# flysoaryun/LF-VIO

Measured on AMD Instinct MI355X. Metric: sliding-window solves/sec (10 KF x N landmarks), higher is better.
Workload: dtype f64; 1 GPU; window300; landmarks=300, observations=1419, windows_per_gpu=1, marginalization=MARGIN_OLD, parallelism=1 independent window stream(s), one per GPU, no data-path collective

## Files before the change

### lf-vio_amd/csrc/kernels_marg.h

```cpp
#pragma once
#include "kernels_solve.h"

constexpr int MARG_THREADS = 768;
constexpr int MARG_MAXD = 96;
constexpr int LDN = 80;
constexpr double JACOBI_TOL = 1e-19;
constexpr size_t MARG_LDS = (size_t)19072 * sizeof(double);
constexpr int BT_GROUP = 4;

DEV void gauge_landmarks(Slot *S, int l0) {
  const int l = l0 + (int)threadIdx.x;
  double *lam = S->lam[S->tr.cur];
  if (l < S->N) lam[l] = 1.0 / (1.0 / lam[l]);
}
template <class T>
DEV void copy_rounds(T *dst, const T *src, int n, int tid, int nthr) {
  for (int k0 = tid; k0 < n; k0 += 8 * nthr) {
    T v[8];
#pragma unroll
    for (int q = 0; q < 8; q++) v[q] = src[k0 + q * nthr < n ? k0 + q * nthr : 0];
#pragma unroll
    for (int q = 0; q < 8; q++)
      if (k0 + q * nthr < n) dst[k0 + q * nthr] = v[q];
  }
}
DEV void gauge_poses(Slot *S, int gated, bool publish);
DEV void publish_solution(Slot *S) {
  char *m = (char *)S->mail;
  if (!m) return;
  const int tid = threadIdx.x, nthr = blockDim.x;
  const TRState *ts = &S->tr;
  const int cur = ts->cur, N = S->N;
  {
    constexpr int XW = (int)(sizeof(FrameState) / 8), XT = (XW + 63) / 64, LT = (SPEC_MAX_LM + 63) / 64, TT = 8;
    const double *xs = (const double *)&S->x[cur];
    double *xd = (double *)(m + MAIL_X + (size_t)cur * sizeof(FrameState));
    const long long *tsrc = (const long long *)ts;
    long long *tdst = (long long *)(m + MAIL_TR);
    const int tl = ts->trace_len < LFVIO_MAX_TRACE ? ts->trace_len : LFVIO_MAX_TRACE;
    const int words = (int)((offsetof(TRState, trace) + (size_t)(tl > 0 ? tl : 0) * sizeof(LfvioIterationSummary)) / 8);
    const double *ls = S->lam[cur];
// ... 426 lines not shown
  unsigned cnt = (unsigned)__double2hiint(p) >> 31;
  unsigned bits = (unsigned)__double2hiint(p) >> 31;
  double d0[8], e0[8], d1[8], e1[8];
#pragma unroll
  for (int u = 0; u < 8; u++) d0[u] = Tg[1 + u], e0[u] = Tg[96 + u];
  for (int i0 = 1; i0 < n; i0 += 16) {
    STURM_TOUCH8(d0);
    STURM_TOUCH8(e0);
#pragma unroll
    for (int u = 0; u < 8; u++) d1[u] = Tg[i0 + 8 + u], e1[u] = Tg[96 + i0 + 8 + u - 1];
#pragma unroll
    for (int u = 0; u < 8; u++) {
      const double pn = fma(d0[u] - sigma, p, -e0[u] * pm);
      bits = __builtin_amdgcn_alignbit(bits, (unsigned)__double2hiint(pn), 31);
      pm = p, p = pn;
    }
    STURM_TOUCH8(d1);
    STURM_TOUCH8(e1);
#pragma unroll
    for (int u = 0; u < 8; u++) d0[u] = Tg[i0 + 16 + u], e0[u] = Tg[96 + i0 + 16 + u - 1];
#pragma unroll
    for (int u = 0; u < 8; u++) {
      const double pn = fma(d1[u] - sigma, p, -e1[u] * pm);
      bits = __builtin_amdgcn_alignbit(bits, (unsigned)__double2hiint(pn), 31);
      pm = p, p = pn;
    }
    cnt += __builtin_popcount((bits ^ (bits >> 1)) & 0xffffu);
    const int ex = ilogb(fmax(fmax(fabs(p), fabs(pm)), 1e-300));
    p = ldexp(p, -ex), pm = ldexp(pm, -ex);
  }
  return (int)cnt;
}
struct TriCtx {
  double *dd, *ee, *tau, *vb0, *vb1, *pp, *RV;
  int n, r0, c0;
};
template <int P>
DEV void tri_finish_row(const TriCtx &tc, int kk, const double (&row)[5], bool own) {
  const int n = tc.n, c0 = tc.c0;
  double *vb = (kk & 1) ? tc.vb1 : tc.vb0;
  double a_part = 0.0, ss_part = 0.0, dk = 0.0;
  bool has_d = false;
#pragma unroll
  for (int q = P; q < 5; q++) {
    const int C = c0 + 16 * q;
    if (C == kk) dk = row[q], has_d = true;
    if (C == kk + 1) a_part = row[q];
    if (C > kk + 1 && C < n) ss_part = fma(row[q], row[q], ss_part);
  }
  if (own && has_d) tc.dd[kk] = dk;
  if (kk + 2 >= n) {
    if (own && kk == n - 2 && c0 == ((n - 1) & 15)) tc.ee[kk] = a_part;
    return;
  }
  a_part = sum8(a_part), ss_part = sum8(ss_part);
  const double alpha = a_part + dpp_f64<0x140>(a_part), ss = ss_part + dpp_f64<0x140>(ss_part);
  const double nn = fma(alpha, alpha, ss);
  const bool live = ss > 0.0;
  const double rs = fast_rsqrt(live ? nn : 1.0);
  const double beta = live ? -copysign(nn * rs, alpha) : alpha;
  const double t = live ? (beta - alpha) * -copysign(rs, alpha) : 0.0;
  const double scal = live ? fast_rcp(alpha - beta) : 0.0;
  if (own) {
#pragma unroll
    for (int q = P; q < 5; q++) {
      const int C = c0 + 16 * q;
      const double v = C == kk + 1 ? 1.0 : ((C > kk + 1 && C < n) ? row[q] * scal : 0.0);
      vb[C] = v;
      if (C > kk && C < n) tc.RV[kk * 76 + C - kk - 1] = v;
    }
    if (c0 == 0) tc.tau[kk] = t, tc.ee[kk] = beta;
  }
}
template <int P>
DEV void tri_matvec(const TriCtx &tc, int k, const double (&ar)[5][5], double (&vj)[5]) {
  const double *vb = (k & 1) ? tc.vb1 : tc.vb0;
  const double t = tc.tau[k];
#pragma unroll
  for (int q = P; q < 5; q++) vj[q] = vb[tc.c0 + 16 * q];
  double sacc[5];
#pragma unroll
  for (int i = P; i < 5; i++) {
    sacc[i] = 0.0;
#pragma unroll
    for (int q = P; q < 5; q++) sacc[i] = fma(ar[i][q], vj[q], sacc[i]);
  }
#pragma unroll
  for (int i = P; i < 5; i++) sacc[i] += dpp_f64<0xB1>(sacc[i]);
#pragma unroll
  for (int i = P; i < 5; i++) sacc[i] += dpp_f64<0x4E>(sacc[i]);
#pragma unroll
  for (int i = P; i < 5; i++) sacc[i] += dpp_f64<0x141>(sacc[i]);
#pragma unroll
  for (int i = P; i < 5; i++) sacc[i] += dpp_f64<0x140>(sacc[i]);
  if (tc.c0 == 0) {
#pragma unroll
    for (int i = P; i < 5; i++) tc.pp[tc.r0 + 16 * i] = tc.r0 + 16 * i > k ? t * sacc[i] : 0.0;
  }
}
template <int P>
DEV void tri_update(const TriCtx &tc, int k, double (&ar)[5][5], const double (&vj)[5]) {
  const double *vb = (k & 1) ? tc.vb1 : tc.vb0;
  const double t = tc.tau[k];
  double pj[5], vi[5], pi[5], pvs = 0.0;
#pragma unroll
  for (int q = P; q < 5; q++) pj[q] = tc.pp[tc.c0 + 16 * q];
#pragma unroll
  for (int i = P; i < 5; i++) vi[i] = vb[tc.r0 + 16 * i], pi[i] = tc.pp[tc.r0 + 16 * i];
#pragma unroll
  for (int q = P; q < 5; q++) pvs = fma(pj[q], vj[q], pvs);
  pvs = sum8(pvs);
  pvs += dpp_f64<0x140>(pvs);
  const double K2 = t * pvs;
#pragma unroll
  for (int i = P; i < 5; i++) {
#pragma unroll
    for (int q = P; q < 5; q++) ar[i][q] = fma(-pi[i], vj[q], fma(-vi[i], pj[q], ar[i][q]));
  }
#pragma unroll
  for (int i = P; i < 5; i++) {
    const double kv = K2 * vi[i];
#pragma unroll
    for (int q = P; q < 5; q++) ar[i][q] = fma(kv, vj[q], ar[i][q]);
    if (i == P) tri_finish_row<P>(tc, k + 1, ar[P], tc.r0 == ((k + 1) & 15));
  }
}
template <int QM, int NR>
DEV void bt_apply(const double *RV, const double *tau, int k, int n, int l8, double (&zz)[10]) {
  double vq[NR][10], tk[NR];
#pragma unroll
  for (int r = 0; r < NR; r++) {
    const int kr = k - r;
    const double *v = RV + kr * 76 - (kr + 1);
    tk[r] = tau[kr];
#pragma unroll
    for (int q = QM; q < 10; q++) {
      const int i = l8 + 8 * q;
      if (QM == 0) vq[r][q] = (i > kr && i < n) ? v[i] : 0.0;
      else vq[r][q] = (q > QM || i > kr) ? v[i] : 0.0;
    }
  }
#pragma unroll
  for (int r = 0; r < NR; r++) {
    double s0 = 0.0, s1 = 0.0;
#pragma unroll
    for (int q = QM; q < 10; q++) {
      if ((q - QM) & 1) s1 = fma(vq[r][q], zz[q], s1);
      else s0 = fma(vq[r][q], zz[q], s0);
    }
    const double s = sum8(s0 + s1) * tk[r];
#pragma unroll
    for (int q = QM; q < 10; q++) zz[q] = fma(-s, vq[r][q], zz[q]);
  }
}
template <int NR>
DEV void bt_dispatch(const double *RV, const double *tau, int k, int n, int l8, double (&zz)[10]) {
  switch (k >> 3) {
    case 0: bt_apply<0, NR>(RV, tau, k, n, l8, zz); break;
    case 1: bt_apply<1, NR>(RV, tau, k, n, l8, zz); break;
    case 2: bt_apply<2, NR>(RV, tau, k, n, l8, zz); break;
    case 3: bt_apply<3, NR>(RV, tau, k, n, l8, zz); break;
    case 4: bt_apply<4, NR>(RV, tau, k, n, l8, zz); break;
    case 5: bt_apply<5, NR>(RV, tau, k, n, l8, zz); break;
    case 6: bt_apply<6, NR>(RV, tau, k, n, l8, zz); break;
    case 7: bt_apply<7, NR>(RV, tau, k, n, l8, zz); break;
    case 8: bt_apply<8, NR>(RV, tau, k, n, l8, zz); break;
    default: bt_apply<9, NR>(RV, tau, k, n, l8, zz); break;
  }
}
DEV double guard_pivot(double q, double pivmin) { return copysign(fmax(fabs(q), pivmin), q); }
template <bool SPEC>
DEV bool eig_tridiag(double *A, const double *b, int n, int tid, double *RV, double *DM, double *vec, double *scr, double *nn2, double *Tglob, LfvioPrior *out, double eps, long long *dbg,
                     SpecPoll *sp_) {
  SpecPoll *const sp = SPEC ? sp_ : nullptr;
  const bool poller = SPEC && tid == MARG_THREADS - 1;
#define ESTAMP(k) do { if (tid == 0) dbg[k] = (long long)__builtin_readcyclecounter(); } while (0)
  ESTAMP(26);
  const int wave = tid >> 6, lane = tid & 63;
  double *dd = vec, *ee = vec + 96, *ee2 = vec + 192, *tau = vec + 288, *lam = vec + 384, *pp = vec + 480, *nrm = vec + 576;
  const bool tri = tid < 256;
  const int r0 = (tid >> 4) & 15, c0 = tid & 15;
  double ar[5][5];
#pragma unroll
  for (int i = 0; i < 5; i++)
#pragma unroll
    for (int q = 0; q < 5; q++) {
      const int R = r0 + 16 * i, C = c0 + 16 * q;
      ar[i][q] = (tri && R < n && C < n) ? A[max(R, C) * LDN + min(R, C)] : 0.0;
    }
  double *vb0 = lam, *vb1 = nrm;
  if (tid < 96) dd[tid] = 0.0, ee[tid] = 0.0, ee2[tid] = 0.0, tau[tid] = 0.0, vb0[tid] = 0.0, vb1[tid] = 0.0;
  for (int e = tid; e < 76 * 76; e += MARG_THREADS) RV[e] = 0.0;
  __syncthreads();
  TriCtx tc = {dd, ee, tau, vb0, vb1, pp, RV, n, r0, c0};
  if (tri) tri_finish_row<0>(tc, 0, ar[0], r0 == 0);
  __syncthreads();
  for (int k = 0; k + 2 < n; k++) {
    const int P = (k + 1) >> 4;
    double vj[5];
    if (poller) {
      if ((k & 7) == 0) spec_poll_issue(*sp);
      else if ((k & 7) == 6) spec_poll_take(*sp);
    }
#ifdef LFVIO_TRI_PROFILE
#define TSTAMP(j) do { if (tid == 0 && k == LFVIO_TRI_PROFILE) dbg[3 + j] = (long long)__builtin_readcyclecounter(); } while (0)
#else
#define TSTAMP(j) do { } while (0)
#endif
    TSTAMP(0);
    if (tri) {
      switch (P) {
        case 0: tri_matvec<0>(tc, k, ar, vj); break;
        case 1: tri_matvec<1>(tc, k, ar, vj); break;
        case 2: tri_matvec<2>(tc, k, ar, vj); break;
        case 3: tri_matvec<3>(tc, k, ar, vj); break;
        default: tri_matvec<4>(tc, k, ar, vj); break;
      }
    }
    TSTAMP(1);
    __syncthreads();
    TSTAMP(2);
    if (tri) {
      switch (P) {
        case 0: tri_update<0>(tc, k, ar, vj); break;
        case 1: tri_update<1>(tc, k, ar, vj); break;
        case 2: tri_update<2>(tc, k, ar, vj); break;
        case 3: tri_update<3>(tc, k, ar, vj); break;
        default: tri_update<4>(tc, k, ar, vj); break;
      }
    }
    TSTAMP(3);
    __syncthreads();
    TSTAMP(4);
    if (sp && (k & 7) == 6 && *sp->flag) return true;
  }
  if (tri) {
#pragma unroll
    for (int i = 0; i < 5; i++)
#pragma unroll
      for (int q = 0; q < 5; q++)
        if (r0 + 16 * i == n - 1 && c0 + 16 * q == n - 1) dd[n - 1] = ar[i][q];
  }
  if (poller) spec_poll_issue(*sp);
  __syncthreads();
  ESTAMP(27);
  if (tid < n) ee2[tid] = ee[tid] * ee[tid];
  {
    double lo = 1e300, hi = -1e300;
    if (tid < n) {
      const double r = (tid > 0 ? fabs(ee[tid - 1]) : 0.0) + (tid + 1 < n ? fabs(ee[tid]) : 0.0);
      lo = dd[tid] - r, hi = dd[tid] + r;
    }
    lo = -wave_max(-lo), hi = wave_max(hi);
    if (lane == 0) scr[wave] = lo, scr[16 + wave] = hi;
  }
  __syncthreads();
  double gl = fmin(scr[0], scr[1]), gu = fmax(scr[16], scr[17]);
  {
    const double tn = fmax(fabs(gl), fabs(gu));
    gl -= 2.2e-16 * tn * n + 1e-300, gu += 2.2e-16 * tn * n + 1e-300;
  }
  if (tid < 96) Tglob[tid] = tid < n ? dd[tid] : gu + 1.0, Tglob[96 + tid] = tid + 1 < n ? ee[tid] * ee[tid] : 0.0;
  __threadfence();
  __syncthreads();
  __builtin_amdgcn_s_dcache_inv();
  const unsigned long long ta = (unsigned long long)Tglob;
  unsigned tlo = __builtin_amdgcn_readfirstlane((unsigned)ta), thi = __builtin_amdgcn_readfirstlane((unsigned)(ta >> 32));
  asm volatile("" : "+s"(tlo), "+s"(thi));
  sdouble *Tg = (sdouble *)(((unsigned long long)thi << 32) | tlo);
  {
    const double pivmin = 1e-290;
    const int g3 = lane == 63 ? 20 : lane / 3, l8 = lane == 63 ? 3 : lane - 3 * g3;
    const int m = wave * 21 + g3;
    const int mm = m < n ? m : n - 1;
    {
      int *cntg = (int *)pp;
      double *blo = nn2, *bhi = nn2 + 96;
      const double step = (gu - gl) * (1.0 / 257.0);
      if (tid < 96) blo[tid] = gl, bhi[tid] = gu;
      if (tid < 256) cntg[tid] = sturm_count(Tg, n, gl + step * (double)(tid + 1));
      __syncthreads();
      if (tid <= 256) {
        const int c0 = tid > 0 ? cntg[tid - 1] : 0, c1 = tid < 256 ? cntg[tid] : n;
        const double a = tid > 0 ? gl + step * (double)tid : gl, b = tid < 256 ? gl + step * (double)(tid + 1) : gu;
        for (int e = max(c0, 0); e < min(c1, n); e++) blo[e] = a, bhi[e] = b;
      }
      __syncthreads();
    }
    double lo = nn2[mm], hi = nn2[96 + mm];
    if (tid < 256)
      for (int round = 0; round < 23; round++) {
        const double w = hi - lo;
        const double sigma = lo + w * (double)(l8 < 3 ? l8 + 1 : 1) * 0.25;
        const int cnt = sturm_count(Tg, n, sigma);
        const int f1 = cnt <= mm ? 1 : 0;
        const unsigned long long bal = __ballot(f1);
        const int f = __builtin_popcount((unsigned)(bal >> (3 * g3)) & 7u);
        const double nlo = f == 0 ? lo : lo + w * (double)f * 0.25, nhi = f == 3 ? hi : lo + w * (double)(f + 1) * 0.25;
        lo = nlo, hi = nhi;
      }
    if (tid < 256 && m < n && l8 == 0) lam[m] = 0.5 * (lo + hi);
    if (poller) spec_poll_take(*sp), spec_poll_issue(*sp);
    __syncthreads();
    ESTAMP(28);
    if (sp && *sp->flag) return true;
    const int set = tid >> 7, me = tid & 127;
    const bool work = set < 2 && me < n;
    const int mec = work ? me : 0;
    const double l = lam[mec];
    if (work && set == 0) {
      double q = dd[0] - l;
      A[mec] = q;
      for (int i0 = 1; i0 < n; i0 += 8) {
        double dv[8], ev[8], qs[8];
#pragma unroll
        for (int u = 0; u < 8; u++) dv[u] = dd[i0 + u], ev[u] = ee2[i0 + u - 1];
#pragma unroll
        for (int u = 0; u < 8; u++) {
          q = fma(-ev[u], fast_rcp(guard_pivot(q, pivmin)), dv[u] - l);
          qs[u] = q;
        }
#pragma unroll
        for (int u = 0; u < 8; u++)
// ... 59 lines not shown
            zs[u] = z;
            nn = on ? fma(z, z, nn) : nn;
          }
#pragma unroll
          for (int u = 0; u < 8; u++)
            if (i0 - u < kt && i0 - u >= 0) A[(i0 - u) * LDN + mec] = zs[u];
        }
      } else {
        for (int i0 = 1; i0 < n; i0 += 8) {
          double c[8], zs[8];
#pragma unroll
          for (int u = 0; u < 8; u++) {
            const int i = min(i0 + u, n - 1);
            c[u] = -ee[i - 1] * fast_rcp(guard_pivot(DM[i * LDN + mec], pivmin));
          }
#pragma unroll
          for (int u = 0; u < 8; u++) {
            const bool on = i0 + u > kt && i0 + u < n;
            z = on ? c[u] * z : 1.0;
            zs[u] = z;
            nn = on ? fma(z, z, nn) : nn;
          }
#pragma unroll
          for (int u = 0; u < 8; u++)
            if (i0 + u > kt && i0 + u < n) A[(i0 + u) * LDN + mec] = zs[u];
        }
      }
      nn2[set * 96 + mec] = nn;
    }
  }
  __syncthreads();
  ESTAMP(29);
  {
    const int m = tid >> 3, l8 = tid & 7;
    const bool live = m < n;
    const int mm = live ? m : 0;
    double zz[10];
    const double sc = fast_rsqrt(1.0 + nn2[mm] + nn2[96 + mm]);
#pragma unroll
    for (int q = 0; q < 10; q++) {
      const int i = l8 + 8 * q;
      zz[q] = i < n ? A[i * LDN + mm] * sc : 0.0;
    }
    int k = n - 3;
    for (; k >= 0 && (k & (BT_GROUP - 1)) != BT_GROUP - 1; k--) bt_dispatch<1>(RV, tau, k, n, l8, zz);
    for (; k >= 0; k -= BT_GROUP) bt_dispatch<BT_GROUP>(RV, tau, k, n, l8, zz);
    const double l = lam[mm];
    double rb = 0.0;
#pragma unroll
    for (int q = 0; q < 10; q++) {
      const int i = l8 + 8 * q;
      if (i < n) rb = fma(zz[q], b[i], rb);
    }
    rb = sum8(rb);
    if (live) {
      const bool keep = l > eps;
      const double sq = keep ? sqrt(l) : 0.0;
#pragma unroll
      for (int q = 0; q < 10; q++) {
        const int i = l8 + 8 * q;
        if (i < n) out->linearized_jacobians[m * n + i] = sq * zz[q];
      }
      if (l8 == 0) out->linearized_residuals[m] = keep ? rb / sq : 0.0;
    }
  }
  return false;
}

DEV void spec_deliver(Slot *S, Slot *S0, int my_word, bool publish) {
  const int tid = threadIdx.x, nthr = blockDim.x;
  __shared__ int give;
  if (tid == 0) {
    const int ep = spec_ep(my_word), a = spec_acc(my_word);
    long long t0 = wall_clock64();
    int g = 0;
    for (;;) {
      const int f = spec_peek(&S0->spec.fin), w = spec_peek(&S0->spec.word);
      if (spec_ep(w) != ep) break;
      const int st = spec_ep(f) == ep ? spec_fin_state(f) : FIN_OPEN;
      if (st >= FIN_MAIN) {
        g = st == FIN_SIDE && spec_fin_acc(f) == a;
        break;
      }
      if (w != my_word) break;
      if (wall_clock64() - t0 > SPEC_WAIT_TICKS) {
        if (spec_cas(&S0->spec.own[a], SPEC_SIDE, SPEC_ABANDON) == SPEC_SIDE) break;
        t0 = wall_clock64();
      }
      __builtin_amdgcn_s_sleep(8);
    }
    give = g;
  }
  __syncthreads();
  if (!give) return;
  const LfvioPrior *src = &S->prior_out;
  LfvioPrior *dst = &S0->prior_out;
// ... 18 lines not shown
  const int publish = (flag_bits >> 10) & 1;
  constexpr bool worker = WORKER;
  Slot *S = worker ? (Slot *)base : SLOT(base, stride);
  Slot *S0 = worker ? (Slot *)(base - stride) : S;
  __shared__ int spec_flag;
  SpecPoll sp{S0, worker ? S->shadow.word : 0, &spec_flag, 0, 0};
  if (threadIdx.x == 0) spec_flag = 0;
  const bool poller = worker && threadIdx.x == MARG_THREADS - 1;
  TRState *tr = &S->tr;
  const MargPlan *mp = &S->marg[flag];
  const int tid = threadIdx.x;
  LfvioPrior *out = &S->prior_out;
  if (gated && !tail_gate(S, tr->done)) return;
  if (worker && sp.my_word == 0) return;
  if (!mp->valid) {
    if (tid == 0) out->valid = -1;
    if (worker) {
      __syncthreads();
      spec_deliver(S, S0, sp.my_word, publish != 0);
      return;
    }
    if (gated && tid == 0) S->iters_done = tr->iteration, S->tail_state = 2;
    if (gated && publish) {
      __syncthreads();
      publish_prior(S);
    }
    return;
  }
  if (poller) spec_poll_issue(sp);
  STAMP(S, 10);
  const double *Sc = S->schur_sum;
  const bool sub = mp->N0 > 0 || S->sharded;
  const int m15 = mp->m15, n = mp->n, D = m15 + n;
  double *Ag = S->mscr;
  double *A = smem;
  double *bv = A + 92 * 92;
  double *Am = bv + 96;
  double *Vm = Am + 256;
  double *Ainv = Vm + 256;
  double *Tm = Ainv + 256;
  double *Ar = smem + 12544;
  double *br = Ar + 76 * LDN;
  double2 *cs = (double2 *)(br + 80);
  int *perm = (int *)(cs + 96);
  double *scr = (double *)(perm + 96);
  double *RV = smem, *vec8 = smem + 5776, *DMs = smem + 5776 + 672;
  for (int c = tid; c < KP; c += MARG_THREADS) {
    const int a = mp->col[c];
    if (a >= 0) perm[a] = c;
  }
  __syncthreads();
  {
    constexpr int GR = (92 * 92 + MARG_THREADS - 1) / MARG_THREADS;
    const double *Hp = &S->Hpp[0];
    double hv[GR], sv[GR];
#pragma unroll
    for (int k = 0; k < GR; k++) {
      const int e = tid + MARG_THREADS * k, ec = e < D * D ? e : 0;
      const int r = D ? perm[ec / max(D, 1)] : 0, c = D ? perm[ec % max(D, 1)] : 0;
      const int hi = max(r, c), lo = min(r, c);
      hv[k] = Hp[hi * (hi + 1) / 2 + lo];
      sv[k] = (sub && hi < KC) ? Sc[schur_index(lo, hi)] : 0.0;
    }
#pragma unroll
    for (int k = 0; k < GR; k++) {
      const int e = tid + MARG_THREADS * k;
      if (e < D * D) A[e] = hv[k] - sv[k];
// ... 45 lines not shown
  }
  __syncthreads();
  {
    const int nb4 = (n + 3) >> 2;
    for (int blk = tid; blk < nb4 * nb4; blk += MARG_THREADS) {
      const int r0 = 4 * (blk / nb4), c0 = 4 * (blk % nb4);
      double acc[4][4];
#pragma unroll
      for (int i = 0; i < 4; i++)
#pragma unroll
        for (int j = 0; j < 4; j++) acc[i][j] = 0.0;
      for (int k = 0; k < m15; k++) {
        double tv[4], av[4];
#pragma unroll
        for (int i = 0; i < 4; i++) tv[i] = Tm[min(r0 + i, n - 1) * m15 + k], av[i] = A[k * D + m15 + min(c0 + i, n - 1)];
#pragma unroll
        for (int i = 0; i < 4; i++)
#pragma unroll
          for (int j = 0; j < 4; j++) acc[i][j] = fma(tv[i], av[j], acc[i][j]);
      }
#pragma unroll
      for (int i = 0; i < 4; i++)
#pragma unroll
        for (int j = 0; j < 4; j++)
          if (r0 + i < n && c0 + j < n) Ar[(r0 + i) * LDN + c0 + j] = A[(m15 + r0 + i) * D + m15 + c0 + j] - acc[i][j];
    }
  }
  for (int r = tid; r < n; r += MARG_THREADS) {
    double s = 0;
    for (int k = 0; k < m15; k++) s = fma(Tm[r * m15 + k], bv[k], s);
    br[r] = bv[m15 + r] - s;
  }
  __syncthreads();
  double *Aout = Ag + 92 * 92 + 96;
  for (int e = tid; e < n * n; e += MARG_THREADS) {
    const int r = e / n, c = e % n;
    Aout[e] = Ar[max(r, c) * LDN + min(r, c)];
  }
  for (int r = tid; r < n; r += MARG_THREADS) Aout[n * n + r] = br[r];
  if (poller) spec_poll_take(sp);
  __syncthreads();
  if (worker && spec_flag) return;
  STAMP(S, 13);
  if (eig_tridiag<WORKER>(Ar, br, n, tid, RV, DMs, vec8, scr, (double *)cs, S->eig_aux, out, 1e-8, S->dbg, &sp)) return;
  if (tid == 0) S->dbg[24] = sw1;
  STAMP(S, 14);
  const FrameState *x = &S->x[tr->cur];
  if (tid < mp->nb) {
    const int kind = mp->kind[tid], frame = mp->frame[tid];
    out->blocks[tid].kind = kind;
    out->blocks[tid].frame = mp->shifted_frame[tid];
    out->block_idx[tid] = mp->idx[tid];
    const double *xb = kind == LFVIO_BLOCK_POSE ? x->pose[frame]
                       : kind == LFVIO_BLOCK_SPEEDBIAS ? x->sb[frame]
                       : kind == LFVIO_BLOCK_EX_POSE ? x->ex
                                                     : &x->td;
    const int gs = (kind == LFVIO_BLOCK_POSE || kind == LFVIO_BLOCK_EX_POSE) ? 7 : (kind == LFVIO_BLOCK_SPEEDBIAS ? 9 : 1);
    for (int k = 0; k < 9; k++) out->block_x0[tid][k] = k < gs ? xb[k] : 0.0;
  }
  STAMP(S, 15);
  if (tid == 0) {
    out->valid = 1;
    out->m = m15 + (S->sharded ? (int)(S->xch[XOFF_C + XS_N0] + 0.5) : mp->N0);
    out->n = n;
    out->num_blocks = mp->nb;
    if (gated && !worker) S->iters_done = tr->iteration, S->tail_state = 2;
  }
  if (worker) {
    __syncthreads();
    spec_deliver(S, S0, sp.my_word, publish != 0);
    return;
  }
  if (gated && publish) {
    __syncthreads();
    publish_prior(S);
  }
}
```

### lf-vio_amd/csrc/lfvio_hip.hip

```cpp
#include <hip/hip_runtime.h>
#include <dlfcn.h>
typedef struct ncclComm *ncclComm_t;
#define NCCL_UNIQUE_ID_BYTES 128
typedef struct {
  char internal[NCCL_UNIQUE_ID_BYTES];
} ncclUniqueId;
typedef int ncclResult_t;
typedef int ncclDataType_t;
typedef int ncclRedOp_t;
constexpr ncclResult_t ncclSuccess = 0;
constexpr ncclRedOp_t ncclSum = 0;
constexpr ncclDataType_t ncclDouble = 8;

#include <algorithm>
#include <chrono>
#include <cmath>
#include <cstdio>
#include <cstdlib>
#include <cstring>
#include <memory>
#include <string>
#include <type_traits>
#include <vector>

// ... 1849 lines not shown
  if ((rc = upload_window(c, 0, in))) return rc;
  const Route r = route_for(c, 1, MODE_SOLVE);
  char *d = c->d_base;
  const size_t o_tr = offsetof(Slot, tr);
  auto poke_int = [&](size_t off, int v) { return hipMemcpy(d + o_tr + off, &v, sizeof v, hipMemcpyHostToDevice); };
  auto run = [&](int do_lin, std::vector<double> &out) -> int {
    HIPCHK(c, hipMemcpy(d + o_tr + offsetof(TRState, mu), &mu, sizeof mu, hipMemcpyHostToDevice));
    HIPCHK(c, poke_int(offsetof(TRState, do_lin), do_lin));
    HIPCHK(c, poke_int(offsetof(TRState, do_schur), 1));
    launch_sweep(c, r, MODE_SOLVE, true);
    HIPCHK(c, hipGetLastError());
    HIPCHK(c, hipStreamSynchronize(c->stream));
    out.resize(SCHUR_LEN);
    HIPCHK(c, hipMemcpy(out.data(), d + c->L.xch + sizeof(double) * XOFF_S, sizeof(double) * SCHUR_LEN, hipMemcpyDeviceToHost));
    return LFVIO_OK;
  };
  launch_setup(c, r, MODE_SOLVE);
  HIPCHK(c, hipStreamSynchronize(c->stream));
  std::vector<double> first, repeat, full;
  const double mu1 = mu;
  mu = 1e-8;
  if ((rc = run(1, first))) return rc;
  launch_solve(c, 1, r.sweep == Route::LINW);
  HIPCHK(c, hipStreamSynchronize(c->stream));
  mu = mu1;
  if ((rc = run(0, repeat))) return rc;
  if ((rc = run(1, full))) return rc;
  double m = 0, ref = 0;
  for (int i = 0; i < SCHUR_LEN; i++) m = std::max(m, std::fabs(repeat[i] - full[i])), ref = std::max(ref, std::fabs(full[i] - first[i]));
  *max_abs_diff = m;
  return ref > 0 ? LFVIO_OK : LFVIO_ERR_ARG;
}

int lfvio_debug_marg_system(lfvio_ctx *c, int n, double *A, double *b) {
  if (!c || !c->d_base) return LFVIO_ERR_ARG;
  (void)hipSetDevice(c->device);
  if (int rc = join_inflight(c)) return rc;
  if (n < 0 || n > 76) return LFVIO_ERR_ARG;
  if (n == 0) return LFVIO_OK;
  char *d = c->d_base + c->L.mscr;
  if (c->shadow) {
    const size_t head = offsetof(LfvioPrior, linearized_jacobians), bytes = head + sizeof(double) * n * n;
    std::vector<char> p0(bytes), pw(bytes);
    HIPCHK(c, hipMemcpy(p0.data(), c->d_base + offsetof(Slot, prior_out), bytes, hipMemcpyDeviceToHost));
    const LfvioPrior *h0 = (const LfvioPrior *)p0.data();
    for (int wk = 0; wk < lfvio_ctx::WORKERS && h0->valid == 1 && h0->n == n; wk++) {
      char *ds = c->d_base + (size_t)(c->batch + wk) * c->L.total;
      HIPCHK(c, hipMemcpy(pw.data(), ds + offsetof(Slot, prior_out), bytes, hipMemcpyDeviceToHost));
      const LfvioPrior *hw = (const LfvioPrior *)pw.data();
      if (hw->valid == 1 && hw->n == n && std::memcmp(p0.data() + head, pw.data() + head, bytes - head) == 0) {
        d = ds + c->L.mscr;
        break;
      }
    }
  }
  HIPCHK(c, hipMemcpy(A, d + sizeof(double) * (92 * 92 + 96), sizeof(double) * n * n, hipMemcpyDeviceToHost));
  HIPCHK(c, hipMemcpy(b, d + sizeof(double) * (92 * 92 + 96 + n * n), sizeof(double) * n, hipMemcpyDeviceToHost));
  return LFVIO_OK;
}

int lfvio_debug_read_clocks(lfvio_ctx *c, long long *out32) {
  if (!c || !c->d_base) return LFVIO_ERR_ARG;
  if (int rc = join_inflight(c)) return rc;
  HIPCHK(c, hipMemcpy(out32, c->d_base + offsetof(Slot, dbg), sizeof(long long) * 32, hipMemcpyDeviceToHost));
  HIPCHK(c, hipMemcpy(out32 + 32, c->d_base + offsetof(Slot, jtrace), sizeof(double) * 32, hipMemcpyDeviceToHost));
  return LFVIO_OK;
}

int lfvio_debug_time_kernel(lfvio_ctx *c, int which, int count, int reps, double *avg_ms) {
  if (!c || !c->d_base || count <= 0 || count > c->batch || reps <= 0) return LFVIO_ERR_ARG;
  (void)hipSetDevice(c->device);
  if (int rc = join_inflight(c)) return rc;
  const Route r = route_for(c, count, MODE_SOLVE);
  const Grid &g = r.g;
  const size_t st = c->L.total;
  const bool lw = r.sweep == Route::LINW, lb = r.sweep == Route::LINB;
  const bool offs = (r.offs & 2) != 0;
  if ((which == 11 || which == 12) && !lw) {
    c->err = "the resident windows are not linearized by k_linw";
    return LFVIO_ERR_ARG;
  }
  if (which >= 15 && which <= 17 && !lb) {
    c->err = "the resident window is not linearized by k_linb";
    return LFVIO_ERR_ARG;
  }
  hipEvent_t e0, e1;
  HIPCHK(c, hipEventCreate(&e0));
  if (hipError_t e = hipEventCreate(&e1); e != hipSuccess) {
    (void)hipEventDestroy(e0);
    HIPCHK(c, e);
// ... 106 lines not shown
  else if (k == "linw") {
    if (iv < 0 || iv > 2) return LFVIO_ERR_ARG;
    c->linw_mode = iv;
  } else if (k == "lm_half") c->lm_half = iv != 0;
  else if (k == "force_eig") c->force_eig = iv != 0;
  else if (k == "marg_ahead") c->marg_ahead = iv != 0;
  else if (k == "break_next_chain") c->debug_break_chain = iv != 0;
  else if (k == "relo_route") c->relo_force = iv != 0;
  else {
    c->err = "lfvio_debug_configure: unknown key '" + k + "'";
    return LFVIO_ERR_ARG;
  }
  if (structural) destroy_graph(c);
  return LFVIO_OK;
}

int lfvio_debug_query(lfvio_ctx *c, const char *key, double *out, int n) {
  if (!c || !key || !out || n <= 0) return LFVIO_ERR_ARG;
  const std::string k = key;
  auto put = [&](std::initializer_list<double> v) {
    int i = 0;
    for (double x : v)
      if (i < n) out[i++] = x;
    return LFVIO_OK;
  };
  if (k == "last_call") return put({(double)c->last_passes, (double)c->last_iters, (double)c->stat_chunks, (double)c->spec_count});
  if (k == "marg_ahead") return put({(double)c->stat_ahead_calls, (double)c->stat_ahead_hits});
  if (k == "upload_times") return put({c->up_us[0], c->up_us[1], c->up_us[2], c->up_us[3]});
  if (k == "sweep_kernel") {
    const int r = sweep_kernel_of(c, (int)out[0]);
    if (r < 0) return r;
    return put({(double)r});
  }
  c->err = "lfvio_debug_query: unknown key '" + k + "'";
  return LFVIO_ERR_ARG;
}

#include "relo.inc"
#include "feat.inc"

#include "twoview.inc"

#include "vialign.inc"

#include "pnp.inc"
#include "shard.inc"
#include "group.inc"

}
```

### lf-vio_amd/lfvio/engine.py

```python
import ctypes as C

import numpy as np

from . import abi

_dp = C.POINTER(C.c_double)


def _p(a):
    return a.ctypes.data_as(_dp)


class Engine:
    def __init__(self, device=0, lib_path=None):
        self.lib = abi.load_hip_library(lib_path)
        self.lib.lfvio_debug_linearize.argtypes = [C.c_void_p, C.POINTER(abi.WindowC), _dp, _dp, _dp, _dp, _dp, _dp]
        self.lib.lfvio_debug_marg_system.argtypes = [C.c_void_p, C.c_int, _dp, _dp]
        self.lib.lfvio_debug_configure.argtypes = [C.c_void_p, C.c_char_p, C.c_double]
        self.lib.lfvio_debug_query.argtypes = [C.c_void_p, C.c_char_p, _dp, C.c_int]
        self.lib.lfvio_debug_time_kernel.argtypes = [C.c_void_p, C.c_int, C.c_int, C.c_int, _dp]
        self.ctx = self.lib.lfvio_create(device)
        if not self.ctx:
            raise RuntimeError("lfvio_create failed: no usable HIP device (there is no CPU fallback)")

# ... 68 lines not shown
    def solve(self, win):
        sol = abi.Solution(win.N)
        self._check(self.lib.lfvio_solve(self.ctx, C.byref(win.c()), C.byref(sol.c)), "lfvio_solve")
        return sol

    def solve_relo(self, win, frame, relo_pose, landmark=(), match_point=()):
        relo = abi.Relo(frame, relo_pose, landmark, match_point)
        rc_ = relo.c()
        sol = abi.Solution(win.N)
        out = np.zeros(abi.SIZE_POSE)
        self._check(self.lib.lfvio_solve_relo(self.ctx, C.byref(win.c()), C.byref(rc_), C.byref(sol.c), _p(out)), "lfvio_solve_relo")
        return sol, out

    def solve_relo_rc(self, win, relo, sol, out, num_matches=None, null_arrays=False):
        rc_ = relo.c(num_matches=num_matches, null_arrays=null_arrays)
        return int(self.lib.lfvio_solve_relo(self.ctx, C.byref(win.c()), C.byref(rc_), C.byref(sol.c), _p(out)))

    def marginalize(self, win, flag):
        prior = abi.Prior()
        self._check(self.lib.lfvio_marginalize(self.ctx, C.byref(win.c()), flag, C.byref(prior)), "lfvio_marginalize")
        return prior

    def schur_repeat(self, win, mu):
        d = np.zeros(1)
        self.lib.lfvio_debug_schur_repeat.argtypes = [C.c_void_p, C.POINTER(abi.WindowC), C.c_double, _dp]
        self._check(self.lib.lfvio_debug_schur_repeat(self.ctx, C.byref(win.c()), float(mu), _p(d)), "lfvio_debug_schur_repeat")
        return float(d[0])

    def marg_system(self, n):
        A = np.zeros((n, n))
        b = np.zeros(n)
        self._check(self.lib.lfvio_debug_marg_system(self.ctx, n, _p(A), _p(b)), "lfvio_debug_marg_system")
        return A, b

    def linearize(self, win):
        N = win.N
        H = np.zeros((abi.KP, abi.KP))
        g = np.zeros(abi.KP)
        a, b = np.zeros(max(N, 1)), np.zeros(max(N, 1))
        W = np.zeros((max(N, 1), abi.KC))
        cost = np.zeros(1)
        self._check(self.lib.lfvio_debug_linearize(self.ctx, C.byref(win.c()), _p(H), _p(g), _p(a), _p(b), _p(W),
                                                   _p(cost)), "lfvio_debug_linearize")
        return dict(H=H, g=g, a=a[:N], b=b[:N], W=W[:N], cost=float(cost[0]))

    def batch_reserve(self, batch, max_landmarks, max_observations):
        self._check(self.lib.lfvio_batch_reserve(self.ctx, batch, max_landmarks, max_observations), "batch_reserve")

    def batch_upload(self, slot, win, marshalled=None):
        self._check(self.lib.lfvio_batch_upload(self.ctx, slot, C.byref(marshalled if marshalled is not None else win.c())), "batch_upload")

    def batch_upload_chained(self, slot, win, prior, marshalled=None):
        self._check(self.lib.lfvio_batch_upload_chained(self.ctx, slot, C.byref(marshalled if marshalled is not None else win.c()), C.byref(prior)),
                    "batch_upload_chained")

    def set_first_passes(self, n):
        self.configure("first_passes", int(n))

    def batch_upload_chained_device(self, slot, win, marshalled=None):
        self._check(self.lib.lfvio_batch_upload_chained_device(self.ctx, slot, C.byref(marshalled if marshalled is not None else win.c())),
                    "batch_upload_chained_device")

    def batch_optimize(self, count, flag, sync=True):
        fn = self.lib.lfvio_batch_optimize if sync else self.lib.lfvio_batch_optimize_async
        self._check(fn(self.ctx, count, flag), "batch_optimize")

# ... 321 lines not shown
```

Baseline: 2402 solves/s.

## Accumulate explicit Q during tridiagonalization and back-transform eigenvectors with MFMA

Idle threads (tid>=256) now build the orthogonal Q matrix explicitly alongside the Householder tridiagonal reduction, applying each reflector while the tri threads do their matvec and update. The serial per-reflector back-transformation of eigenvectors is replaced by a dense Q*Z product using f64 MFMA 16x16x4 tiles spread over all waves. The residual reduction is done through a per-tile partial-sum buffer. The global scratch copy of A and b and the block metadata writes are moved into the otherwise idle bisection phase. In exchange this adds register pressure and DPP reductions for the Q-update threads, plus a new debug query for Q.

```diff
diff --git a/lf-vio_amd/csrc/kernels_marg.h b/lf-vio_amd/csrc/kernels_marg.h
--- a/lf-vio_amd/csrc/kernels_marg.h
+++ b/lf-vio_amd/csrc/kernels_marg.h
@@ -3,10 +3,10 @@
 
 constexpr int MARG_THREADS = 768;
 constexpr int MARG_MAXD = 96;
+constexpr int MARG_GQ = 0, MARG_GA = 92 * 92 + 96;
 constexpr int LDN = 80;
 constexpr double JACOBI_TOL = 1e-19;
 constexpr size_t MARG_LDS = (size_t)19072 * sizeof(double);
-constexpr int BT_GROUP = 4;
 
 DEV void gauge_landmarks(Slot *S, int l0) {
   const int l = l0 + (int)threadIdx.x;
@@ -499,7 +499,7 @@
   return (int)cnt;
 }
 struct TriCtx {
-  double *dd, *ee, *tau, *vb0, *vb1, *pp, *RV;
+  double *dd, *ee, *tau, *vb0, *vb1, *pp;
   int n, r0, c0;
 };
 template <int P>
@@ -534,7 +534,6 @@
       const int C = c0 + 16 * q;
       const double v = C == kk + 1 ? 1.0 : ((C > kk + 1 && C < n) ? row[q] * scal : 0.0);
       vb[C] = v;
-      if (C > kk && C < n) tc.RV[kk * 76 + C - kk - 1] = v;
     }
     if (c0 == 0) tc.tau[kk] = t, tc.ee[kk] = beta;
   }
@@ -592,53 +591,43 @@
     if (i == P) tri_finish_row<P>(tc, k + 1, ar[P], tc.r0 == ((k + 1) & 15));
   }
 }
-template <int QM, int NR>
-DEV void bt_apply(const double *RV, const double *tau, int k, int n, int l8, double (&zz)[10]) {
-  double vq[NR][10], tk[NR];
-#pragma unroll
-  for (int r = 0; r < NR; r++) {
-    const int kr = k - r;
-    const double *v = RV + kr * 76 - (kr + 1);
-    tk[r] = tau[kr];
-#pragma unroll
-    for (int q = QM; q < 10; q++) {
-      const int i = l8 + 8 * q;
-      if (QM == 0) vq[r][q] = (i > kr && i < n) ? v[i] : 0.0;
-      else vq[r][q] = (q > QM || i > kr) ? v[i] : 0.0;
-    }
-  }
-#pragma unroll
-  for (int r = 0; r < NR; r++) {
-    double s0 = 0.0, s1 = 0.0;
-#pragma unroll
-    for (int q = QM; q < 10; q++) {
-      if ((q - QM) & 1) s1 = fma(vq[r][q], zz[q], s1);
-      else s0 = fma(vq[r][q], zz[q], s0);
-    }
-    const double s = sum8(s0 + s1) * tk[r];
-#pragma unroll
-    for (int q = QM; q < 10; q++) zz[q] = fma(-s, vq[r][q], zz[q]);
-  }
-}
-template <int NR>
-DEV void bt_dispatch(const double *RV, const double *tau, int k, int n, int l8, double (&zz)[10]) {
-  switch (k >> 3) {
-    case 0: bt_apply<0, NR>(RV, tau, k, n, l8, zz); break;
-    case 1: bt_apply<1, NR>(RV, tau, k, n, l8, zz); break;
-    case 2: bt_apply<2, NR>(RV, tau, k, n, l8, zz); break;
-    case 3: bt_apply<3, NR>(RV, tau, k, n, l8, zz); break;
-    case 4: bt_apply<4, NR>(RV, tau, k, n, l8, zz); break;
-    case 5: bt_apply<5, NR>(RV, tau, k, n, l8, zz); break;
-    case 6: bt_apply<6, NR>(RV, tau, k, n, l8, zz); break;
-    case 7: bt_apply<7, NR>(RV, tau, k, n, l8, zz); break;
-    case 8: bt_apply<8, NR>(RV, tau, k, n, l8, zz); break;
-    default: bt_apply<9, NR>(RV, tau, k, n, l8, zz); break;
-  }
+template <int P>
+DEV void q_dot(const TriCtx &tc, int k, const double (&qr)[5][5], double (&vj)[5], double (&s)[3]) {
+  const double *vb = (k & 1) ? tc.vb1 : tc.vb0;
+  const double t = tc.tau[k];
+#pragma unroll
+  for (int q = P; q < 5; q++) {
+    const double v = vb[tc.c0 + 16 * q];
+    vj[q] = tc.c0 + 16 * q > k ? v : 0.0;
+  }
+#pragma unroll
+  for (int i = 0; i < 3; i++) {
+    s[i] = 0.0;
+#pragma unroll
+    for (int q = P; q < 5; q++) s[i] = fma(qr[i][q], vj[q], s[i]);
+  }
+#pragma unroll
+  for (int i = 0; i < 3; i++) s[i] += dpp_f64<0xB1>(s[i]);
+#pragma unroll
+  for (int i = 0; i < 3; i++) s[i] += dpp_f64<0x4E>(s[i]);
+#pragma unroll
+  for (int i = 0; i < 3; i++) s[i] += dpp_f64<0x141>(s[i]);
+#pragma unroll
+  for (int i = 0; i < 3; i++) s[i] += dpp_f64<0x140>(s[i]);
+#pragma unroll
+  for (int i = 0; i < 3; i++) s[i] *= t;
+}
+template <int P>
+DEV void q_update(double (&qr)[5][5], const double (&vj)[5], const double (&s)[3]) {
+#pragma unroll
+  for (int i = 0; i < 3; i++)
+#pragma unroll
+    for (int q = P; q < 5; q++) qr[i][q] = fma(-s[i], vj[q], qr[i][q]);
 }
 DEV double guard_pivot(double q, double pivmin) { return copysign(fmax(fabs(q), pivmin), q); }
-template <bool SPEC>
+template <bool SPEC, class Side>
 DEV bool eig_tridiag(double *A, const double *b, int n, int tid, double *RV, double *DM, double *vec, double *scr, double *nn2, double *Tglob, LfvioPrior *out, double eps, long long *dbg,
-                     SpecPoll *sp_) {
+                     SpecPoll *sp_, double *gscr, Side side) {
   SpecPoll *const sp = SPEC ? sp_ : nullptr;
   const bool poller = SPEC && tid == MARG_THREADS - 1;
 #define ESTAMP(k) do { if (tid == 0) dbg[k] = (long long)__builtin_readcyclecounter(); } while (0)
@@ -646,25 +635,25 @@
   const int wave = tid >> 6, lane = tid & 63;
   double *dd = vec, *ee = vec + 96, *ee2 = vec + 192, *tau = vec + 288, *lam = vec + 384, *pp = vec + 480, *nrm = vec + 576;
   const bool tri = tid < 256;
-  const int r0 = (tid >> 4) & 15, c0 = tid & 15;
+  const int r0 = (tid >> 4) & 15, c0 = tid & 15, qg = (tid - 256) >> 4;
   double ar[5][5];
 #pragma unroll
   for (int i = 0; i < 5; i++)
 #pragma unroll
     for (int q = 0; q < 5; q++) {
       const int R = r0 + 16 * i, C = c0 + 16 * q;
-      ar[i][q] = (tri && R < n && C < n) ? A[max(R, C) * LDN + min(R, C)] : 0.0;
+      if (tri) ar[i][q] = (R < n && C < n) ? A[max(R, C) * LDN + min(R, C)] : 0.0;
+      else ar[i][q] = (i < 3 && qg + 32 * i == C && C < n) ? 1.0 : 0.0;
     }
   double *vb0 = lam, *vb1 = nrm;
   if (tid < 96) dd[tid] = 0.0, ee[tid] = 0.0, ee2[tid] = 0.0, tau[tid] = 0.0, vb0[tid] = 0.0, vb1[tid] = 0.0;
-  for (int e = tid; e < 76 * 76; e += MARG_THREADS) RV[e] = 0.0;
-  __syncthreads();
-  TriCtx tc = {dd, ee, tau, vb0, vb1, pp, RV, n, r0, c0};
+  __syncthreads();
+  TriCtx tc = {dd, ee, tau, vb0, vb1, pp, n, r0, c0};
   if (tri) tri_finish_row<0>(tc, 0, ar[0], r0 == 0);
   __syncthreads();
   for (int k = 0; k + 2 < n; k++) {
     const int P = (k + 1) >> 4;
-    double vj[5];
+    double vj[5], qs[3];
     if (poller) {
       if ((k & 7) == 0) spec_poll_issue(*sp);
       else if ((k & 7) == 6) spec_poll_take(*sp);
@@ -683,6 +672,14 @@
         case 3: tri_matvec<3>(tc, k, ar, vj); break;
         default: tri_matvec<4>(tc, k, ar, vj); break;
       }
+    } else {
+      switch (P) {
+        case 0: q_dot<0>(tc, k, ar, vj, qs); break;
+        case 1: q_dot<1>(tc, k, ar, vj, qs); break;
+        case 2: q_dot<2>(tc, k, ar, vj, qs); break;
+        case 3: q_dot<3>(tc, k, ar, vj, qs); break;
+        default: q_dot<4>(tc, k, ar, vj, qs); break;
+      }
     }
     TSTAMP(1);
     __syncthreads();
@@ -695,6 +692,14 @@
         case 3: tri_update<3>(tc, k, ar, vj); break;
         default: tri_update<4>(tc, k, ar, vj); break;
       }
+    } else {
+      switch (P) {
+        case 0: q_update<0>(ar, vj, qs); break;
+        case 1: q_update<1>(ar, vj, qs); break;
+        case 2: q_update<2>(ar, vj, qs); break;
+        case 3: q_update<3>(ar, vj, qs); break;
+        default: q_update<4>(ar, vj, qs); break;
+      }
     }
     TSTAMP(3);
     __syncthreads();
@@ -707,6 +712,14 @@
 #pragma unroll
       for (int q = 0; q < 5; q++)
         if (r0 + 16 * i == n - 1 && c0 + 16 * q == n - 1) dd[n - 1] = ar[i][q];
+  } else {
+#pragma unroll
+    for (int i = 0; i < 3; i++)
+#pragma unroll
+      for (int q = 0; q < 5; q++) {
+        const int R = qg + 32 * i, C = c0 + 16 * q;
+        if (R < n && C < n) RV[R * 76 + C] = ar[i][q];
+      }
   }
   if (poller) spec_poll_issue(*sp);
   __syncthreads();
@@ -755,7 +768,17 @@
       __syncthreads();
     }
     double lo = nn2[mm], hi = nn2[96 + mm];
-    if (tid < 256)
+    if (tid >= 256) {
+      if (wave == 4) side(lane);
+      const int t = tid - 256;
+      double *Qg = gscr + MARG_GQ, *Aout = gscr + MARG_GA;
+      const int c = t & 127;
+      for (int r = t >> 7; r < n && c < n; r += 4) {
+        Qg[r * n + c] = RV[r * 76 + c];
+        Aout[r * n + c] = A[max(r, c) * LDN + min(r, c)];
+      }
+      if (t < n) Qg[76 * 76 + t] = dd[t], Qg[76 * 76 + 96 + t] = t + 1 < n ? ee[t] : 0.0, Aout[n * n + t] = b[t];
+    } else
       for (int round = 0; round < 23; round++) {
         const double w = hi - lo;
         const double sigma = lo + w * (double)(l8 < 3 ? l8 + 1 : 1) * 0.25;
@@ -881,36 +904,52 @@
   __syncthreads();
   ESTAMP(29);
   {
-    const int m = tid >> 3, l8 = tid & 7;
-    const bool live = m < n;
-    const int mm = live ? m : 0;
-    double zz[10];
-    const double sc = fast_rsqrt(1.0 + nn2[mm] + nn2[96 + mm]);
-#pragma unroll
-    for (int q = 0; q < 10; q++) {
-      const int i = l8 + 8 * q;
-      zz[q] = i < n ? A[i * LDN + mm] * sc : 0.0;
-    }
-    int k = n - 3;
-    for (; k >= 0 && (k & (BT_GROUP - 1)) != BT_GROUP - 1; k--) bt_dispatch<1>(RV, tau, k, n, l8, zz);
-    for (; k >= 0; k -= BT_GROUP) bt_dispatch<BT_GROUP>(RV, tau, k, n, l8, zz);
-    const double l = lam[mm];
-    double rb = 0.0;
-#pragma unroll
-    for (int q = 0; q < 10; q++) {
-      const int i = l8 + 8 * q;
-      if (i < n) rb = fma(zz[q], b[i], rb);
-    }
-    rb = sum8(rb);
-    if (live) {
-      const bool keep = l > eps;
-      const double sq = keep ? sqrt(l) : 0.0;
-#pragma unroll
-      for (int q = 0; q < 10; q++) {
-        const int i = l8 + 8 * q;
-        if (i < n) out->linearized_jacobians[m * n + i] = sq * zz[q];
-      }
-      if (l8 == 0) out->linearized_residuals[m] = keep ? rb / sq : 0.0;
+    typedef double d4 __attribute__((ext_vector_type(4)));
+    const int nt = (n + 15) >> 4, nk = (n + 3) >> 2;
+    const int lr = lane & 15, lq = lane >> 4;
+    double *part = DM;
+    for (int t = wave; t < nt * nt; t += MARG_THREADS / 64) {
+      const int tm = t / nt, ti = t - tm * nt;
+      const int m = 16 * tm + lr, i = 16 * ti + lr;
+      const bool mv = m < n, iv = i < n;
+      const int mc = mv ? m : 0, ic = iv ? i : 0;
+      const double sc = fast_rsqrt(1.0 + nn2[mc] + nn2[96 + mc]);
+      d4 acc = {0.0, 0.0, 0.0, 0.0};
+      for (int kb = 0; kb < nk; kb += 5) {
+        double z[5], qv[5];
+#pragma unroll
+        for (int u = 0; u < 5; u++) {
+          const int k = 4 * (kb + u) + lq;
+          const bool kv = k < n;
+          const int kc = kv ? k : 0;
+          z[u] = (mv && kv) ? A[kc * LDN + mc] * sc : 0.0;
+          qv[u] = (iv && kv) ? RV[ic * 76 + kc] : 0.0;
+        }
+#pragma unroll
+        for (int u = 0; u < 5; u++) acc = __builtin_amdgcn_mfma_f64_16x16x4f64(z[u], qv[u], acc, 0, 0, 0);
+      }
+      const double bi = iv ? b[ic] : 0.0;
+#pragma unroll
+      for (int r = 0; r < 4; r++) {
+        const int mr = 16 * tm + lq + 4 * r;
+        const bool live = mr < n;
+        const double l = lam[live ? mr : 0];
+        const double sq = l > eps ? sqrt(l) : 0.0;
+        if (live && iv) out->linearized_jacobians[mr * n + i] = sq * acc[r];
+        double p = acc[r] * bi;
+        p += dpp_f64<0xB1>(p);
+        p += dpp_f64<0x4E>(p);
+        p += dpp_f64<0x141>(p);
+        p += dpp_f64<0x140>(p);
+        if (live && lr == 0) part[ti * 96 + mr] = p;
+      }
+    }
+    __syncthreads();
+    if (tid < n) {
+      double rb = 0.0;
+      for (int ti = 0; ti < nt; ti++) rb += part[ti * 96 + tid];
+      const double l = lam[tid];
+      out->linearized_residuals[tid] = l > eps ? rb / sqrt(l) : 0.0;
     }
   }
   return false;
@@ -995,7 +1034,6 @@
   const double *Sc = S->schur_sum;
   const bool sub = mp->N0 > 0 || S->sharded;
   const int m15 = mp->m15, n = mp->n, D = m15 + n;
-  double *Ag = S->mscr;
   double *A = smem;
   double *bv = A + 92 * 92;
   double *Am = bv + 96;
@@ -1107,32 +1145,30 @@
     br[r] = bv[m15 + r] - s;
   }
   __syncthreads();
-  double *Aout = Ag + 92 * 92 + 96;
-  for (int e = tid; e < n * n; e += MARG_THREADS) {
-    const int r = e / n, c = e % n;
-    Aout[e] = Ar[max(r, c) * LDN + min(r, c)];
-  }
-  for (int r = tid; r < n; r += MARG_THREADS) Aout[n * n + r] = br[r];
   if (poller) spec_poll_take(sp);
   __syncthreads();
   if (worker && spec_flag) return;
   STAMP(S, 13);
-  if (eig_tridiag<WORKER>(Ar, br, n, tid, RV, DMs, vec8, scr, (double *)cs, S->eig_aux, out, 1e-8, S->dbg, &sp)) return;
+  const FrameState *x = &S->x[tr->cur];
+  auto blocks = [&](int b) {
+    if (b < mp->nb) {
+      const int kind = mp->kind[b], frame = mp->frame[b];
+      out->blocks[b].kind = kind;
+      out->blocks[b].frame = mp->shifted_frame[b];
+      out->block_idx[b] = mp->idx[b];
+      const double *xb = kind == LFVIO_BLOCK_POSE ? x->pose[frame]
+                         : kind == LFVIO_BLOCK_SPEEDBIAS ? x->sb[frame]
+                         : kind == LFVIO_BLOCK_EX_POSE ? x->ex
+                                                       : &x->td;
+      const int gs = (kind == LFVIO_BLOCK_POSE || kind == LFVIO_BLOCK_EX_POSE) ? 7 : (kind == LFVIO_BLOCK_SPEEDBIAS ? 9 : 1);
+      for (int k = 0; k < 9; k++) out->block_x0[b][k] = k < gs ? xb[k] : 0.0;
+    }
+  };
+  if (n == 0) {
+    if (tid < 64) blocks(tid);
+  } else if (eig_tridiag<WORKER>(Ar, br, n, tid, RV, DMs, vec8, scr, (double *)cs, S->eig_aux, out, 1e-8, S->dbg, &sp, S->mscr, blocks)) return;
   if (tid == 0) S->dbg[24] = sw1;
   STAMP(S, 14);
-  const FrameState *x = &S->x[tr->cur];
-  if (tid < mp->nb) {
-    const int kind = mp->kind[tid], frame = mp->frame[tid];
-    out->blocks[tid].kind = kind;
-    out->blocks[tid].frame = mp->shifted_frame[tid];
-    out->block_idx[tid] = mp->idx[tid];
-    const double *xb = kind == LFVIO_BLOCK_POSE ? x->pose[frame]
-                       : kind == LFVIO_BLOCK_SPEEDBIAS ? x->sb[frame]
-                       : kind == LFVIO_BLOCK_EX_POSE ? x->ex
-                                                     : &x->td;
-    const int gs = (kind == LFVIO_BLOCK_POSE || kind == LFVIO_BLOCK_EX_POSE) ? 7 : (kind == LFVIO_BLOCK_SPEEDBIAS ? 9 : 1);
-    for (int k = 0; k < 9; k++) out->block_x0[tid][k] = k < gs ? xb[k] : 0.0;
-  }
   STAMP(S, 15);
   if (tid == 0) {
     out->valid = 1;
diff --git a/lf-vio_amd/csrc/lfvio_hip.hip b/lf-vio_amd/csrc/lfvio_hip.hip
--- a/lf-vio_amd/csrc/lfvio_hip.hip
+++ b/lf-vio_amd/csrc/lfvio_hip.hip
@@ -1905,12 +1905,7 @@
   return ref > 0 ? LFVIO_OK : LFVIO_ERR_ARG;
 }
 
-int lfvio_debug_marg_system(lfvio_ctx *c, int n, double *A, double *b) {
-  if (!c || !c->d_base) return LFVIO_ERR_ARG;
-  (void)hipSetDevice(c->device);
-  if (int rc = join_inflight(c)) return rc;
-  if (n < 0 || n > 76) return LFVIO_ERR_ARG;
-  if (n == 0) return LFVIO_OK;
+static int marg_scratch_of(lfvio_ctx *c, int n, char **scratch) {
   char *d = c->d_base + c->L.mscr;
   if (c->shadow) {
     const size_t head = offsetof(LfvioPrior, linearized_jacobians), bytes = head + sizeof(double) * n * n;
@@ -1927,8 +1922,35 @@
       }
     }
   }
-  HIPCHK(c, hipMemcpy(A, d + sizeof(double) * (92 * 92 + 96), sizeof(double) * n * n, hipMemcpyDeviceToHost));
-  HIPCHK(c, hipMemcpy(b, d + sizeof(double) * (92 * 92 + 96 + n * n), sizeof(double) * n, hipMemcpyDeviceToHost));
+  *scratch = d;
+  return LFVIO_OK;
+}
+
+int lfvio_debug_marg_system(lfvio_ctx *c, int n, double *A, double *b) {
+  if (!c || !c->d_base) return LFVIO_ERR_ARG;
+  (void)hipSetDevice(c->device);
+  if (int rc = join_inflight(c)) return rc;
+  if (n < 0 || n > 76) return LFVIO_ERR_ARG;
+  if (n == 0) return LFVIO_OK;
+  char *d;
+  if (int rc = marg_scratch_of(c, n, &d)) return rc;
+  HIPCHK(c, hipMemcpy(A, d + sizeof(double) * MARG_GA, sizeof(double) * n * n, hipMemcpyDeviceToHost));
+  HIPCHK(c, hipMemcpy(b, d + sizeof(double) * (MARG_GA + n * n), sizeof(double) * n, hipMemcpyDeviceToHost));
+  return LFVIO_OK;
+}
+
+static int marg_q_of(lfvio_ctx *c, double *out, int cap) {
+  if (!c->d_base) return LFVIO_ERR_ARG;
+  (void)hipSetDevice(c->device);
+  if (int rc = join_inflight(c)) return rc;
+  const int n = (int)out[0];
+  if (n < 1 || n > 76 || cap < n * n + 2 * n) return LFVIO_ERR_ARG;
+  char *d;
+  if (int rc = marg_scratch_of(c, n, &d)) return rc;
+  d += sizeof(double) * MARG_GQ;
+  HIPCHK(c, hipMemcpy(out, d, sizeof(double) * n * n, hipMemcpyDeviceToHost));
+  HIPCHK(c, hipMemcpy(out + n * n, d + sizeof(double) * 76 * 76, sizeof(double) * n, hipMemcpyDeviceToHost));
+  HIPCHK(c, hipMemcpy(out + n * n + n, d + sizeof(double) * (76 * 76 + 96), sizeof(double) * n, hipMemcpyDeviceToHost));
   return LFVIO_OK;
 }
 
@@ -2101,6 +2123,7 @@
     if (r < 0) return r;
     return put({(double)r});
   }
+  if (k == "marg_q") return marg_q_of(c, out, n);
   c->err = "lfvio_debug_query: unknown key '" + k + "'";
   return LFVIO_ERR_ARG;
 }
diff --git a/lf-vio_amd/lfvio/engine.py b/lf-vio_amd/lfvio/engine.py
--- a/lf-vio_amd/lfvio/engine.py
+++ b/lf-vio_amd/lfvio/engine.py
@@ -124,6 +124,12 @@
         b = np.zeros(n)
         self._check(self.lib.lfvio_debug_marg_system(self.ctx, n, _p(A), _p(b)), "lfvio_debug_marg_system")
         return A, b
+
+    def marg_q(self, n):
+        out = np.zeros(n * n + 2 * n)
+        out[0] = n
+        self._check(self.lib.lfvio_debug_query(self.ctx, b"marg_q", _p(out), out.size), "lfvio_debug_query(marg_q)")
+        return out[:n * n].reshape(n, n).copy(), out[n * n:n * n + n].copy(), out[n * n + n:n * n + 2 * n - 1].copy()
 
     def linearize(self, win):
         N = win.N
```

Result: slower. 1429 solves/s (-40.5%).
